# quickwit-oss/tantivy

Measured on AMD Instinct MI355X. Metric: queries_per_sec_2term_AND_bm25_top10, higher is better.
Workload: dtype u32+f32; 1 GPU; and2: 10000 queries/batch, k=10, one 10M-doc Zipf segment per GPU (256 terms, df_r=0.5N/r, WithFreqs); term ranks ~ Zipf(1); distinct_queries=3877, mode=block-max pruned (block_wand_intersection semantics), exchange=single rank: no exchange, segments_per_gpu=1, index_bytes=40381332

## Files before the change

### tantivy_amd/csrc/tq_misc.hip

```cpp
#include "tq_common.hpp"

namespace {

template <int KPL, bool PRE>
__global__ __launch_bounds__(64) void merge_kernel(TqkMergeParams p) {
  const int lane = (int)__lane_id();
  const uint32_t q = PRE ? blockIdx.x % p.n_queries : blockIdx.x;
  if (q >= p.n_queries) return;
  const TqdQuery *Q = uni_ptr(p.queries + q);
  const uint32_t k = uni(Q->k);
  uint32_t part_start = uni(Q->part_start), n_parts = uni(Q->n_parts);
  const uint32_t per = tqk_merge_slice_lists(n_parts, p.pre_slices);
  uint32_t stride = 1u;
  if constexpr (PRE) {
    if (per == 1u) return;
    const uint32_t sl = blockIdx.x / p.n_queries;
    if (sl * per >= n_parts) return;
    part_start += sl * per;
    n_parts = n_parts - sl * per < per ? n_parts - sl * per : per;
    if (n_parts == 1u) return;
  } else {
    stride = per;
    n_parts = (n_parts + per - 1u) / per;
  }
  TopK<KPL> tk;
  tk.reset(k);
  uint64_t floor_key = 0;
  for (uint32_t pi = (uint32_t)lane; pi < n_parts; pi += WAVE) {
    const uint64_t kth = p.partials[(uint64_t)(part_start + pi * stride) * (uint64_t)(KPL * 64) + (k - 1u)];
    floor_key = kth > floor_key ? kth : floor_key;
  }
  for (int o = 32; o; o >>= 1) {
    const uint64_t other = ((uint64_t)(uint32_t)__shfl_xor((int)(floor_key >> 32), o, WAVE) << 32) |
                           (uint32_t)__shfl_xor((int)(uint32_t)floor_key, o, WAVE);
    floor_key = other > floor_key ? other : floor_key;
  }
  constexpr uint32_t GROUP = KPL <= 2 ? 8u : (KPL <= 4 ? 4u : 1u);
  for (uint32_t pi0 = 0; pi0 < n_parts; pi0 += GROUP) {
    uint64_t keys[GROUP][KPL];
#pragma unroll
    for (uint32_t g = 0; g < GROUP; ++g) {
      const uint32_t pi = pi0 + g < n_parts ? pi0 + g : n_parts - 1u;
      const uint64_t *src = p.partials + (uint64_t)(part_start + pi * stride) * (uint64_t)(KPL * 64);
#pragma unroll
      for (int r = 0; r < KPL; ++r) keys[g][r] = src[(uint32_t)r * 64u + (uint32_t)lane];
    }
#pragma unroll
    for (uint32_t g = 0; g < GROUP; ++g) {
      if (pi0 + g >= n_parts) break;
#pragma unroll
      for (int r = 0; r < KPL; ++r)
        tk.offer(keys[g][r] != 0ull && keys[g][r] >= floor_key, keys[g][r], lane);
    }
  }
  if constexpr (PRE) {
    flush_partial<KPL>(tk, const_cast<uint64_t *>(p.partials), part_start, lane);
    return;
  }
  const uint32_t out_q = p.out_index ? p.out_index[q] : q;
  uint32_t count = 0;
#pragma unroll
  for (int r = 0; r < KPL; ++r) {
    const uint32_t rank = (uint32_t)r * 64u + (uint32_t)lane;
    const bool real = rank < k && tk.v[r] != 0ull;
    count += (uint32_t)__popcll(__ballot(real));
    if (rank < p.out_stride) {
      p.out_scores[(uint64_t)out_q * p.out_stride + rank] = real ? key_score(tk.v[r]) : 0.0f;
      p.out_docs[(uint64_t)out_q * p.out_stride + rank] = real ? key_doc(tk.v[r]) : TQD_TERMINATED;
    }
  }
  for (uint32_t rank = (uint32_t)(KPL * 64) + (uint32_t)lane; rank < p.out_stride; rank += 64u) {
    p.out_scores[(uint64_t)out_q * p.out_stride + rank] = 0.0f;
    p.out_docs[(uint64_t)out_q * p.out_stride + rank] = TQD_TERMINATED;
  }
  if (lane == 0) p.out_counts[out_q] = count;
}

__global__ __launch_bounds__(256) void zero_regions_kernel(TqkZeroParams p) {
  const uint32_t r = blockIdx.y;
  uint32_t *dst = p.ptr[r];
  const uint32_t n = p.words[r];
  const uint32_t head = (uint32_t)((16u - ((uintptr_t)dst & 15u)) & 15u) >> 2;
  const uint32_t h = head < n ? head : n;
  const uint32_t tid = blockIdx.x * 256u + threadIdx.x, stride = gridDim.x * 256u;
  if (tid < h) dst[tid] = 0u;
  const uint32_t n4 = (n - h) >> 2;
  uint4 *d4 = reinterpret_cast<uint4 *>(dst + h);
  for (uint32_t i = tid; i < n4; i += stride) d4[i] = make_uint4(0u, 0u, 0u, 0u);
  const uint32_t tail0 = h + (n4 << 2);
  if (tid < n - tail0) dst[tail0 + tid] = 0u;
}

template <bool USE_DPP>
__global__ __launch_bounds__(256) void decode_list_kernel(TqdSegment seg, const TqdTerm *terms,
                                                          uint32_t handle, uint32_t *docs,
                                                          uint32_t *tfs) {
  const int lane = (int)__lane_id();
  const uint32_t wave = uni(threadIdx.x >> 6);
  const TermRef t = load_term(terms, handle);
  const uint32_t j = blockIdx.x * 4u + wave;
  if (j >= t.n_blocks) return;
  const Dec d = decode_block<USE_DPP, false>(uni_ptr(seg.idx), t, j, lane);
  const uint32_t i0 = j * 128u + 2u * (uint32_t)lane;
  const uint32_t df = uni(terms[handle].doc_freq);
  if (i0 < df) {
    docs[i0] = d.d0;
    tfs[i0] = d.t0;
  }
  if (i0 + 1u < df) {
    docs[i0 + 1u] = d.d1;
    tfs[i0 + 1u] = d.t1;
  }
}

__global__ void decode_positions_kernel(TqdSegment seg, const TqdTerm *terms, uint32_t handle,
                                        uint32_t *out, uint64_t n) {
  const uint64_t i = (uint64_t)blockIdx.x * blockDim.x + threadIdx.x;
  if (i >= n) return;
  out[i] = position_delta(seg.pos, terms + handle, i);
}

__global__ __launch_bounds__(64) void merge_segments_kernel(TqkSegMergeParams p) {
  const int lane = (int)__lane_id();
  const uint32_t q = blockIdx.x;
  if (q >= p.n_queries) return;
  const uint32_t total = p.n_segments * p.stride;
  const uint32_t want = p.offset + p.limit;
  uint32_t n_valid = 0;
  for (uint32_t s = 0; s < p.n_segments; ++s) n_valid += p.counts[(uint64_t)s * p.n_queries + q];
  for (uint32_t c = (uint32_t)lane; c < total; c += 64u) {
    const uint32_t s = c / p.stride, i = c % p.stride;
    const uint32_t cnt = p.counts[(uint64_t)s * p.n_queries + q];
    if (i >= cnt) continue;
    const uint64_t at = ((uint64_t)s * p.n_queries + q) * p.stride + i;
    const float sc = p.scores[at];
    const uint32_t dc = p.docs[at];
    const uint32_t so = p.segment_ords ? p.segment_ords[s] : s;
    uint32_t before = 0;
    for (uint32_t s2 = 0; s2 < p.n_segments; ++s2) {
      const uint32_t cnt2 = p.counts[(uint64_t)s2 * p.n_queries + q];
      const uint32_t so2 = p.segment_ords ? p.segment_ords[s2] : s2;
      const uint64_t b2 = ((uint64_t)s2 * p.n_queries + q) * p.stride;
      for (uint32_t i2 = 0; i2 < cnt2; ++i2) {
        const float sc2 = p.scores[b2 + i2];
        const uint32_t dc2 = p.docs[b2 + i2];
        const bool lt = (sc2 > sc) || (sc2 == sc && (so2 < so || (so2 == so && dc2 < dc)));
        before += lt ? 1u : 0u;
      }
    }
    if (before >= p.offset && before < want) {
      const uint64_t o = (uint64_t)q * p.limit + (before - p.offset);
      p.out_scores[o] = sc;
      p.out_segment_ords[o] = so;
      p.out_docs[o] = dc;
    }
  }
  const uint32_t got = n_valid > p.offset ? (n_valid - p.offset < p.limit ? n_valid - p.offset : p.limit) : 0u;
  for (uint32_t r = got + (uint32_t)lane; r < p.limit; r += 64u) {
    const uint64_t o = (uint64_t)q * p.limit + r;
    p.out_scores[o] = 0.0f;
    p.out_segment_ords[o] = 0xFFFFFFFFu;
    p.out_docs[o] = TQD_TERMINATED;
  }
  if (lane == 0) p.out_counts[q] = got;
}

__global__ void docmat_init_kernel(uint64_t *mat, const uint8_t *fieldnorm, uint32_t const_id,
                                   uint32_t max_doc) {
  const uint32_t d = blockIdx.x * blockDim.x + threadIdx.x;
  if (d < max_doc) mat[d] = fieldnorm ? (uint64_t)fieldnorm[d] : (uint64_t)const_id;
}
__global__ void docmat_set_kernel(uint64_t *mat, const uint32_t *docs, uint32_t n, uint32_t slot,
                                  uint32_t max_doc) {
  const uint32_t i = blockIdx.x * blockDim.x + threadIdx.x;
  if (i < n && docs[i] < max_doc)
    atomicOr((unsigned long long *)(mat + docs[i]), 1ull << (8u + slot));
}

template <bool USE_DPP>
__global__ __launch_bounds__(256) void docsig_batch_kernel(TqdSegment seg, const TqdTerm *const *selfs, const uint32_t *bits,
                                                           uint64_t *mat, uint32_t *const *tabs, const uint32_t *shifts,
                                                           const uint32_t *dfs, const float *cache, uint32_t *lmax_out) {
  const int lane = (int)__lane_id();
  const uint32_t wave = uni(threadIdx.x >> 6);
  const TqdTerm *self = selfs[blockIdx.x];
  const TermRef t = load_term(self, 0u);
  const uint32_t b = bits[blockIdx.x];
  const uint64_t bit = 1ull << (TQD_SIG_SHIFT + (b & 15u));
  const bool sig = mat != nullptr && b != 0xFFFFFFFFu;
  uint32_t *dir = tabs ? tabs[blockIdx.x] : nullptr;
  const uint32_t S = dir ? shifts[blockIdx.x] : 0u, df = dir ? dfs[blockIdx.x] : 0u;
  const uint32_t n_ranges = (seg.max_doc >> S) + 1u;
  uint32_t *ent = dir ? dir + ((n_ranges + 1u + 3u) & ~3u) : nullptr;
  uint32_t lmax = 0;
  for (uint32_t j = wave; j < t.n_blocks; j += 4u) {
    const Dec d = decode_block<USE_DPP, false>(uni_ptr(seg.idx), t, j, lane);
    if (sig) {
      if (d.d0 < seg.max_doc) atomicOr((unsigned long long *)(mat + d.d0), (unsigned long long)bit);
      if (d.d1 < seg.max_doc) atomicOr((unsigned long long *)(mat + d.d1), (unsigned long long)bit);
    }
    if (ent) {
      const uint32_t i0 = 128u * j + 2u * (uint32_t)lane;
      const uint32_t up = (uint32_t)__shfl_up((int)d.d1, 1, WAVE);
      uint32_t r_from = lane ? (up >> S) + 1u : (j ? (block_prev_last(t, j) >> S) + 1u : 0u);
#pragma unroll
      for (int e = 0; e < 2; ++e) {
        const uint32_t doc = e ? d.d1 : d.d0, tf = e ? d.t1 : d.t0, i = i0 + (uint32_t)e;
        if (i < df && doc < seg.max_doc) {
          ent[i] = rdir_entry(doc, tf, S);
          const uint32_t r_to = doc >> S;
          for (uint32_t r = r_from; r <= r_to; ++r) dir[r] = i;
          r_from = r_to + 1u;
          if (i + 1u == df)
            for (uint32_t r = r_from; r <= n_ranges; ++r) dir[r] = df;
          if (cache) {
            const float f = (float)tf;
            const float tfn = f / (f + cache[seg.fieldnorm ? (uint32_t)seg.fieldnorm[doc] : seg.const_fieldnorm_id]);
            uint32_t q = (uint32_t)(tfn * 255.0f) + 1u;
            q = q > 255u ? 255u : q;
            lmax = q > lmax ? q : lmax;
          }
        }
      }
    }
  }
  if (!ent || !cache) return;
  for (int o = 32; o; o >>= 1) {
    const uint32_t other = (uint32_t)__shfl_xor((int)lmax, o, WAVE);
    lmax = other > lmax ? other : lmax;
  }
  if (lane == 0 && lmax) atomicMax(lmax_out + blockIdx.x, lmax);
}
__global__ void rdir_fill_kernel(const uint32_t *docs, const uint32_t *tfs, uint32_t n, uint32_t max_doc, uint32_t *dir,
                                 uint32_t S) {
  const uint32_t i = blockIdx.x * blockDim.x + threadIdx.x;
  if (i >= n) return;
  uint32_t *ent = dir + (((max_doc >> S) + 2u + 3u) & ~3u);
  const uint32_t doc = docs[i];
  if (doc >= max_doc) return;
  ent[i] = rdir_entry(doc, tfs[i], S);
  const uint32_t r_to = doc >> S;
  for (uint32_t r = i ? (docs[i - 1u] >> S) + 1u : 0u; r <= r_to; ++r) dir[r] = i;
  if (i + 1u == n)
    for (uint32_t r = r_to + 1u; r <= (max_doc >> S) + 1u; ++r) dir[r] = n;
}

__global__ void doccls_set_kernel(uint64_t *cls, const uint32_t *docs, const uint32_t *tfs, uint32_t n, uint32_t slot,
                                  uint32_t max_doc) {
  const uint32_t i = blockIdx.x * blockDim.x + threadIdx.x;
  if (i < n && docs[i] < max_doc) {
    const uint32_t tf = tfs[i];
    const uint64_t c = tf >= 3u ? 3ull : (tf ? (uint64_t)tf : 3ull);
    atomicOr((unsigned long long *)(cls + docs[i]), (unsigned long long)(c << (2u * slot)));
  }
}

__global__ void tf8_pack_kernel(const uint32_t *tfs, uint32_t n, uint8_t *out) {
  const uint32_t i = blockIdx.x * blockDim.x + threadIdx.x;
  if (i < n) out[i] = (uint8_t)(tfs[i] < 255u ? tfs[i] : 255u);
}

}

hipError_t tqk_launch_tf8_pack(const uint32_t *tfs, uint32_t n, uint8_t *out, hipStream_t st) {
  if (n == 0) return hipSuccess;
  hipLaunchKernelGGL(tf8_pack_kernel, dim3((n + 255) / 256), dim3(256), 0, st, tfs, n, out);
  return hipGetLastError();
}
hipError_t tqk_launch_docmat_init(uint64_t *mat, const uint8_t *fieldnorm, uint32_t const_id,
                                  uint32_t max_doc, hipStream_t st) {
  if (max_doc == 0) return hipSuccess;
  hipLaunchKernelGGL(docmat_init_kernel, dim3((max_doc + 255) / 256), dim3(256), 0, st, mat,
                     fieldnorm, const_id, max_doc);
  return hipGetLastError();
}
hipError_t tqk_launch_docmat_set(uint64_t *mat, const uint32_t *docs, uint32_t n, uint32_t slot,
                                 uint32_t max_doc, hipStream_t st) {
  if (n == 0) return hipSuccess;
  hipLaunchKernelGGL(docmat_set_kernel, dim3((n + 255) / 256), dim3(256), 0, st, mat, docs, n, slot,
                     max_doc);
  return hipGetLastError();
}
hipError_t tqk_launch_docsig_batch(const TqdSegment &seg, const TqdTerm *const *selfs, const uint32_t *bits, uint32_t n,
                                   uint64_t *mat, uint32_t *const *tabs, const uint32_t *shifts, const uint32_t *dfs,
                                   const float *cache, uint32_t *lmax_out, bool use_dpp, hipStream_t st) {
  if (n == 0) return hipSuccess;
  if (use_dpp)
    hipLaunchKernelGGL((docsig_batch_kernel<true>), dim3(n), dim3(256), 0, st, seg, selfs, bits, mat, tabs, shifts, dfs, cache, lmax_out);
  else
    hipLaunchKernelGGL((docsig_batch_kernel<false>), dim3(n), dim3(256), 0, st, seg, selfs, bits, mat, tabs, shifts, dfs, cache, lmax_out);
  return hipGetLastError();
}
hipError_t tqk_launch_rdir_fill(const uint32_t *docs, const uint32_t *tfs, uint32_t n, uint32_t max_doc, uint32_t *dir,
                                uint32_t S, hipStream_t st) {
  if (n == 0) return hipSuccess;
  hipLaunchKernelGGL(rdir_fill_kernel, dim3((n + 255) / 256), dim3(256), 0, st, docs, tfs, n, max_doc, dir, S);
  return hipGetLastError();
}
hipError_t tqk_launch_doccls_set(uint64_t *cls, const uint32_t *docs, const uint32_t *tfs, uint32_t n, uint32_t slot,
                                 uint32_t max_doc, hipStream_t st) {
  if (n == 0) return hipSuccess;
  hipLaunchKernelGGL(doccls_set_kernel, dim3((n + 255) / 256), dim3(256), 0, st, cls, docs, tfs, n, slot, max_doc);
  return hipGetLastError();
}
hipError_t tqk_launch_zero(const TqkZeroParams &p, hipStream_t st) {
  if (p.n == 0) return hipSuccess;
  uint32_t max_words = 0;
  for (uint32_t i = 0; i < p.n; ++i) max_words = max_words > p.words[i] ? max_words : p.words[i];
  if (max_words == 0) return hipSuccess;
  const uint32_t bx = (max_words / 4u + 2047u) / 2048u;
  hipLaunchKernelGGL(zero_regions_kernel, dim3(bx ? (bx > 256u ? 256u : bx) : 1u, p.n), dim3(256), 0, st, p);
  return hipGetLastError();
}
template <bool PRE>
static void launch_merge_t(const TqkMergeParams &p, int kpl, dim3 grid, dim3 block, hipStream_t st) {
  switch (kpl) {
    case 1: merge_kernel<1, PRE><<<grid, block, 0, st>>>(p); break;
    case 2: merge_kernel<2, PRE><<<grid, block, 0, st>>>(p); break;
    case 4: merge_kernel<4, PRE><<<grid, block, 0, st>>>(p); break;
    default: merge_kernel<16, PRE><<<grid, block, 0, st>>>(p); break;
  }
}
hipError_t tqk_launch_merge(const TqkMergeParams &p, int kpl, hipStream_t st) {
  if (p.n_queries == 0) return hipSuccess;
  const dim3 block(64);
  if (p.pre_slices) {
    launch_merge_t<true>(p, kpl, dim3(p.n_queries * p.pre_slices), block, st);
    const hipError_t e = hipGetLastError();
    if (e != hipSuccess) return e;
  }
  launch_merge_t<false>(p, kpl, dim3(p.n_queries), block, st);
  return hipGetLastError();
}
hipError_t tqk_launch_decode_list(const TqdSegment &seg, const TqdTerm *terms, uint32_t handle,
                                  uint32_t n_blocks, uint32_t *docs, uint32_t *tfs, bool use_dpp,
                                  hipStream_t st) {
  if (n_blocks == 0) return hipSuccess;
  const dim3 grid((n_blocks + 3) / 4), block(256);
  if (use_dpp)
    hipLaunchKernelGGL((decode_list_kernel<true>), grid, block, 0, st, seg, terms, handle, docs, tfs);
  else
    hipLaunchKernelGGL((decode_list_kernel<false>), grid, block, 0, st, seg, terms, handle, docs, tfs);
  return hipGetLastError();
}
hipError_t tqk_launch_decode_positions(const TqdSegment &seg, const TqdTerm *terms,
                                       uint32_t handle, uint32_t *out, uint64_t n,
                                       hipStream_t st) {
  if (n == 0) return hipSuccess;
  hipLaunchKernelGGL(decode_positions_kernel, dim3((unsigned)((n + 255) / 256)), dim3(256), 0, st,
                     seg, terms, handle, out, n);
  return hipGetLastError();
}
hipError_t tqk_launch_merge_segments(const TqkSegMergeParams &p, hipStream_t st) {
  if (p.n_queries == 0) return hipSuccess;
  hipLaunchKernelGGL(merge_segments_kernel, dim3(p.n_queries), dim3(64), 0, st, p);
  return hipGetLastError();
}
```

Baseline: 10.65 million queries/s.

## Tile segment merge across queries in LDS with vectorized coalesced stores

Replaces the one-wave-per-query segment merge with a 256-thread block that handles a tile of up to 32 queries. Per-segment top-k lists are staged in shared memory, ranks are computed there by counting, and results are written back with aligned uint4 stores. The aim is to cut launch and per-block overhead for many small queries and to coalesce global traffic. With one segment per GPU this merge may be a trivial fraction of total time, and the large LDS allocation may limit occupancy.

Result: faster. 11.06 million queries/s (median of 6 runs) (+3.9%).

```diff
diff --git a/tantivy_amd/csrc/tq_misc.hip b/tantivy_amd/csrc/tq_misc.hip
--- a/tantivy_amd/csrc/tq_misc.hip
+++ b/tantivy_amd/csrc/tq_misc.hip
@@ -165,6 +165,102 @@
   if (lane == 0) p.out_counts[q] = got;
 }
 
+constexpr uint32_t kSegMergeThreads = 256;
+constexpr uint32_t kSegMergeLdsWords = 8192;
+constexpr uint32_t kSegMergeTileMax = 32;
+
+inline uint32_t seg_merge_tile(uint32_t n_segments, uint32_t stride, uint32_t limit) {
+  const uint64_t per_q = 2ull * n_segments * stride + n_segments + 3ull * limit + 1ull;
+  const uint64_t t = kSegMergeLdsWords / per_q;
+  return (uint32_t)(t < kSegMergeTileMax ? t : kSegMergeTileMax);
+}
+
+__device__ __forceinline__ void seg_merge_store(uint32_t *dst, const uint32_t *src, uint32_t n, uint32_t tid) {
+  const uint32_t mis = (uint32_t)(((uintptr_t)dst >> 2) & 3u);
+  const uint32_t h = min(n, (4u - mis) & 3u);
+  if (tid < h) dst[tid] = src[tid];
+  const uint32_t n4 = (n - h) >> 2;
+  uint4 *d4 = reinterpret_cast<uint4 *>(dst + h);
+  for (uint32_t i = tid; i < n4; i += kSegMergeThreads) {
+    const uint32_t *s = src + h + 4u * i;
+    d4[i] = make_uint4(s[0], s[1], s[2], s[3]);
+  }
+  const uint32_t t0 = h + (n4 << 2);
+  if (tid < n - t0) dst[t0 + tid] = src[t0 + tid];
+}
+
+__global__ __launch_bounds__(kSegMergeThreads) void merge_segments_tile_kernel(TqkSegMergeParams p, uint32_t qt) {
+  extern __shared__ uint32_t sm[];
+  const uint32_t tid = threadIdx.x;
+  const uint32_t S = p.n_segments, stride = p.stride, limit = p.limit;
+  const uint32_t q0 = blockIdx.x * qt;
+  const uint32_t nq = min(qt, p.n_queries - q0);
+  const uint32_t rows = qt * stride;
+  uint32_t *in_sc = sm;
+  uint32_t *in_dc = in_sc + S * rows;
+  uint32_t *in_ct = in_dc + S * rows;
+  uint32_t *o_sc = in_ct + S * qt;
+  uint32_t *o_so = o_sc + qt * limit;
+  uint32_t *o_dc = o_so + qt * limit;
+  uint32_t *o_ct = o_dc + qt * limit;
+  const uint32_t *g_sc = reinterpret_cast<const uint32_t *>(p.scores);
+  for (uint32_t s = 0; s < S; ++s) {
+    const uint64_t base = ((uint64_t)s * p.n_queries + q0) * stride;
+    for (uint32_t i = tid; i < nq * stride; i += kSegMergeThreads) {
+      in_sc[s * rows + i] = g_sc[base + i];
+      in_dc[s * rows + i] = p.docs[base + i];
+    }
+    if (tid < nq) in_ct[s * qt + tid] = min(p.counts[(uint64_t)s * p.n_queries + q0 + tid], stride);
+  }
+  __syncthreads();
+  const uint32_t total = S * stride, want = p.offset + limit;
+  auto got_of = [&](uint32_t ql) -> uint32_t {
+    uint32_t n_valid = 0;
+    for (uint32_t s = 0; s < S; ++s) n_valid += in_ct[s * qt + ql];
+    return n_valid > p.offset ? (n_valid - p.offset < limit ? n_valid - p.offset : limit) : 0u;
+  };
+  for (uint32_t x = tid; x < nq * total; x += kSegMergeThreads) {
+    const uint32_t ql = x / total, c = x - ql * total;
+    const uint32_t s = c / stride, i = c - s * stride;
+    if (i >= in_ct[s * qt + ql]) continue;
+    const float sc = __uint_as_float(in_sc[s * rows + ql * stride + i]);
+    const uint32_t dc = in_dc[s * rows + ql * stride + i];
+    const uint32_t so = p.segment_ords ? p.segment_ords[s] : s;
+    uint32_t before = 0;
+    for (uint32_t s2 = 0; s2 < S; ++s2) {
+      const uint32_t cnt2 = in_ct[s2 * qt + ql];
+      const uint32_t so2 = p.segment_ords ? p.segment_ords[s2] : s2;
+      const uint32_t b2 = s2 * rows + ql * stride;
+      for (uint32_t i2 = 0; i2 < cnt2; ++i2) {
+        const float sc2 = __uint_as_float(in_sc[b2 + i2]);
+        const uint32_t dc2 = in_dc[b2 + i2];
+        const bool lt = (sc2 > sc) || (sc2 == sc && (so2 < so || (so2 == so && dc2 < dc)));
+        before += lt ? 1u : 0u;
+      }
+    }
+    if (before >= p.offset && before < want) {
+      const uint32_t o = ql * limit + (before - p.offset);
+      o_sc[o] = __float_as_uint(sc);
+      o_so[o] = so;
+      o_dc[o] = dc;
+    }
+  }
+  for (uint32_t x = tid; x < nq * limit; x += kSegMergeThreads) {
+    const uint32_t ql = x / limit, r = x - ql * limit;
+    if (r < got_of(ql)) continue;
+    o_sc[x] = __float_as_uint(0.0f);
+    o_so[x] = 0xFFFFFFFFu;
+    o_dc[x] = TQD_TERMINATED;
+  }
+  if (tid < nq) o_ct[tid] = got_of(tid);
+  __syncthreads();
+  const uint64_t o0 = (uint64_t)q0 * limit;
+  seg_merge_store(reinterpret_cast<uint32_t *>(p.out_scores) + o0, o_sc, nq * limit, tid);
+  seg_merge_store(p.out_segment_ords + o0, o_so, nq * limit, tid);
+  seg_merge_store(p.out_docs + o0, o_dc, nq * limit, tid);
+  seg_merge_store(p.out_counts + q0, o_ct, nq, tid);
+}
+
 __global__ void docmat_init_kernel(uint64_t *mat, const uint8_t *fieldnorm, uint32_t const_id,
                                    uint32_t max_doc) {
   const uint32_t d = blockIdx.x * blockDim.x + threadIdx.x;
@@ -353,6 +449,12 @@
 }
 hipError_t tqk_launch_merge_segments(const TqkSegMergeParams &p, hipStream_t st) {
   if (p.n_queries == 0) return hipSuccess;
-  hipLaunchKernelGGL(merge_segments_kernel, dim3(p.n_queries), dim3(64), 0, st, p);
-  return hipGetLastError();
-}
+  const uint32_t qt = seg_merge_tile(p.n_segments, p.stride, p.limit);
+  if (qt == 0) {
+    hipLaunchKernelGGL(merge_segments_kernel, dim3(p.n_queries), dim3(64), 0, st, p);
+    return hipGetLastError();
+  }
+  const size_t lds = (size_t)qt * (2u * p.n_segments * p.stride + p.n_segments + 3u * p.limit + 1u) * sizeof(uint32_t);
+  hipLaunchKernelGGL(merge_segments_tile_kernel, dim3((p.n_queries + qt - 1) / qt), dim3(kSegMergeThreads), lds, st, p, qt);
+  return hipGetLastError();
+}
```
